# frgfm/Holocron

Measured on NVIDIA H100. Metric: images/sec RepVGG-A0 224^2 bf16 train, higher is better.
Workload: dtype bf16

## Files before the change

holocron_b200/csrc/conv_common.cuh:

```cuda
#pragma once
#include <cuda_runtime.h>
#include <type_traits>
#include "common.cuh"
#include "tc_common.cuh"
#include "tmap.cuh"

namespace conv {

constexpr int kThreads = 384;
constexpr int kConsumers = 256;

__device__ __forceinline__ void consumer_sync() { asm volatile("bar.sync 1, 256;" ::: "memory"); }

struct Ring {
  int stage = 0;
  uint32_t phase = 0;
  __device__ __forceinline__ void next(int n) {
    if (++stage == n) { stage = 0; phase ^= 1; }
  }
  __device__ __forceinline__ static Ring at(int k, int n) { return Ring{k % n, (uint32_t)(k / n) & 1}; }
};

__device__ __forceinline__ void add_residual16(uint4& val, const uint4& rv, bool relu) {
  __nv_bfloat162* a = reinterpret_cast<__nv_bfloat162*>(&val);
  const __nv_bfloat162* b = reinterpret_cast<const __nv_bfloat162*>(&rv);
#pragma unroll
  for (int jj = 0; jj < 4; ++jj) {
    float2 fa = __bfloat1622float2(a[jj]), fb = __bfloat1622float2(b[jj]);
    fa.x += fb.x; fa.y += fb.y;
    if (relu) { fa.x = hb::relu_nan(fa.x); fa.y = hb::relu_nan(fa.y); }
    a[jj] = __floats2bfloat162_rn(fa.x, fa.y);
  }
}

__device__ __forceinline__ void accum_pair(float4& s, const uint8_t* staged) {
  const float2 f = __bfloat1622float2(*reinterpret_cast<const __nv_bfloat162*>(staged));
  s.x += f.x; s.y += f.y; s.z = fmaf(f.x, f.x, s.z); s.w = fmaf(f.y, f.y, s.w);
}
__device__ __forceinline__ float2 fold_stats(const float4* scratch, int rgs, int npairs, int c) {
  const int pr = c >> 1, hi = c & 1;
  float sv = 0.f, qv = 0.f;
  for (int rg = 0; rg < rgs; ++rg) {
    const float4 v = scratch[rg * npairs + pr];
    sv += hi ? v.y : v.x;
    qv += hi ? v.w : v.z;
  }
  return make_float2(sv, qv);
}
__device__ __forceinline__ void store_stats(float* stats, int slot, int Cout, int channel, float2 v) {
  *reinterpret_cast<float2*>(stats + ((size_t)slot * Cout + channel) * 2) = v;
}

template <auto kKernel, typename... Args>
cudaError_t launch(int grid, size_t smem_bytes, cudaStream_t stream, const Args&... args) {
  static const cudaError_t attr =
      cudaFuncSetAttribute(kKernel, cudaFuncAttributeMaxDynamicSharedMemorySize, 227 * 1024);
  if (attr != cudaSuccess) return attr;
  kKernel<<<grid, kThreads, smem_bytes, stream>>>(args...);
  g_hb_launches.fetch_add(1, std::memory_order_relaxed);
  return cudaGetLastError();
}

template <int kStep, int kMax, int W = kStep, typename F>
cudaError_t dispatch_width(int w, F&& f) {
  if (w == W) return f(std::integral_constant<int, W>{});
  if constexpr (W + kStep <= kMax) return dispatch_width<kStep, kMax, W + kStep>(w, f);
  else return cudaErrorInvalidValue;
}

}

int hb_conv_rows_try(const void* x, const void* w, void* y, const float* bias, const void* residual, int N, int H, int W,
                     int Cin, int Cout, int act, int num_ctas, cudaStream_t stream, int nextra, const void* const* xe,
                     const void* const* we, float* stats, int* stat_slots);
int hb_wgrad_rows_try(const void* x, const void* dy, const void* dy1, float* ws, size_t ws_bytes, int N, int H, int W,
                      int Cin, int Cout, int num_ctas, cudaStream_t stream, int* slices_out);
size_t hb_wgrad_rows_workspace_bytes(int N, int H, int W, int Cin, int Cout, int R, int S, int stride, int pad, int dil,
                                     int num_ctas, int has_b1);
```

holocron_b200/csrc/conv_fprop.cu:

```cuda
#include <stdlib.h>
#include "conv_common.cuh"
#include "holocron_b200.h"

namespace {

using namespace tc;
using namespace conv;

constexpr int kBM = 128;
constexpr int kBK = 64;
constexpr int kMmaK = 16;
constexpr int kProducerRegs = 40;
constexpr int kConsumerRegs = 232;
constexpr int kABytes = kBM * kBK * 2;
constexpr int kSmemMax = 227 * 1024;

struct FpropParams {
  int m_total;
  int Ho, Wo;
  int stride, pad_h, pad_w, dil;
  int R, S;
  int Cin, Cout;
  int num_m_tiles, num_n_tiles;
  int cblocks;
// ... 322 lines not shown
  p.e_mode = kext ? 1 : (dual ? 2 : 0);
  const int ce = kext ? a.Ce : (dual ? Cin : 0);
  p.e_cblocks = (ce + kBK - 1) / kBK;
  p.e_ksteps_last = p.e_cblocks ? ((ce - (p.e_cblocks - 1) * kBK) + kMmaK - 1) / kMmaK : 0;
  p.b_stage_bytes = ((BN * 128) + 1023) & ~1023;
  p.out_pitch = (BN < 64 ? BN : 64) * 2 + 16;
  const int out_bytes = ((((kBM * p.out_pitch + 15) & ~15) + kBM * 8) + 1023) & ~1023;
  const int stage_bytes = kABytes + p.b_stage_bytes;
  int stages = (kSmemMax - 1024 - out_bytes - 2 * 8 * (int)sizeof(uint64_t)) / stage_bytes;
  if (stages > 8) stages = 8;
  if (stages < 2) return (int)cudaErrorInvalidValue;
  p.stages = stages;
  p.a_mode = (R == 1 && S == 1 && a.stride == 1 && a.pad_h == 0 && a.pad_w == 0 && a.pad_after_h == 0 &&
              a.pad_after_w == 0) ? 0 : 1;
  p.act = a.act;
  p.y = (__nv_bfloat16*)a.y;
  p.y2 = (__nv_bfloat16*)a.y2;
  p.stats = a.stats; p.stats2 = dual ? a.stats2 : nullptr;
  p.bias = a.bias;
  p.residual = (const __nv_bfloat16*)a.residual;
  p.norm_mean = a.norm_mean; p.norm_rstd = a.norm_rstd; p.norm_wsum = a.norm_wsum;
  if (p.norm_mean && (!p.norm_rstd || !p.norm_wsum || a.scatter)) return (int)cudaErrorInvalidValue;

  CUtensorMap tmA, tmB, tmA2, tmB2;
  int rc = p.a_mode == 0 ? tmap::encode_matrix(&tmA, a.x, p.m_total, Cin, kBM)
                         : tmap::encode_im2col_bf16(&tmA, a.x, a.N, a.H, a.W, Cin, a.pad_h, a.pad_w, R, S, a.dil,
                                                    a.stride, kBK, kBM, CU_TENSOR_MAP_SWIZZLE_128B, a.pad_after_h,
                                                    a.pad_after_w);
  if (rc) return rc;
  if ((rc = tmap::encode_krsc_slab(&tmB, a.w, Cout, R * S, Cin, BN))) return rc;
  tmA2 = tmA; tmB2 = tmB;
  if (kext && (rc = tmap::encode_matrix(&tmA2, a.xe, p.m_total, a.Ce, kBM))) return rc;
  if (p.e_mode && (rc = tmap::encode_krsc_slab(&tmB2, kext ? a.we : a.w2, Cout, 1, ce, BN))) return rc;

  const size_t smem_bytes = (size_t)stages * stage_bytes + out_bytes + 2 * stages * sizeof(uint64_t) + 1024;
  int per_n = grid / p.num_n_tiles;
  if (per_n < 1) per_n = 1;
  if (per_n > p.num_m_tiles) per_n = p.num_m_tiles;
  grid = per_n * p.num_n_tiles;
  if (a.stat_slots) *a.stat_slots = 2 * per_n;
  const bool stats = p.stats || p.stats2;
  return (int)dispatch_width<16, 256>(BN, [&](auto bn) {
    constexpr int kBN = decltype(bn)::value;
    if constexpr (kBN > 128) {
      if (stats) return cudaErrorInvalidValue;
      return launch<conv_fprop_kernel<false, kBN>>(grid, smem_bytes, a.stream, tmA, tmB, tmA2, tmB2, p);
    } else {
      return stats ? launch<conv_fprop_kernel<true, kBN>>(grid, smem_bytes, a.stream, tmA, tmB, tmA2, tmB2, p)
                   : launch<conv_fprop_kernel<false, kBN>>(grid, smem_bytes, a.stream, tmA, tmB, tmA2, tmB2, p);
    }
  });
}

}

extern "C" {

int hb_conv2d_fprop_bf16(const void* x, const void* w, void* y, const float* bias, const void* residual, int N, int H,
                         int W, int Cin, int Cout, int R, int S, int stride, int pad, int dil, int act, int num_ctas,
                         void* stream) {
  hb_conv_args a{};
  a.x = x; a.w = w; a.y = y; a.bias = bias; a.residual = residual;
  a.N = N; a.H = H; a.W = W; a.Cin = Cin; a.Cout = Cout; a.R = R; a.S = S; a.stride = stride; a.pad = pad; a.dil = dil;
  a.act = act; a.num_ctas = num_ctas;
  return hb_conv2d_fused_bf16(&a, nullptr, stream);
}

int hb_conv_stat_slots_max(void) { return 2 * HB_NUM_SMS * 4; }

int hb_conv2d_fused_bf16(const hb_conv_args* c, int* stat_slots, void* stream) {
  if (!c) return (int)cudaErrorInvalidValue;
  const int N = c->N, H = c->H, W = c->W, Cin = c->Cin, Cout = c->Cout, R = c->R, S = c->S;
  const int stride = c->stride, pad = c->pad, dil = c->dil;
  if (Cin % 8 != 0 || Cout % 16 != 0) return (int)cudaErrorInvalidValue;
  if (!hb::aligned16(c->x) || !hb::aligned16(c->w) || !hb::aligned16(c->y)) return (int)cudaErrorMisalignedAddress;
  if (c->w2 && (!hb::aligned16(c->w2) || !hb::aligned16(c->y2))) return (int)cudaErrorMisalignedAddress;
  const int Ho = (H + 2 * pad - dil * (R - 1) - 1) / stride + 1;
  const int Wo = (W + 2 * pad - dil * (S - 1) - 1) / stride + 1;
  if (Ho <= 0 || Wo <= 0) return (int)cudaErrorInvalidValue;
  if ((long long)N * Ho * Wo > 0x7fffffffLL) return (int)cudaErrorInvalidValue;
  if (c->w2 && pad != (R / 2) * dil) return (int)cudaErrorInvalidValue;
  if ((c->stats || c->stats2) && !stat_slots) return (int)cudaErrorInvalidValue;

  if (R == 3 && S == 3 && stride == 1 && pad == 1 && dil == 1 && !c->xe && !c->w2 && !c->norm_mean) {
    static const bool rows_enabled = getenv("HB_DISABLE_CONV_ROWS") == nullptr;
    if (rows_enabled) {
      const int rc = hb_conv_rows_try(c->x, c->w, c->y, c->bias, c->residual, N, H, W, Cin, Cout, c->act, c->num_ctas,
                                      (cudaStream_t)stream, 0, nullptr, nullptr, c->stats, stat_slots);
      if (rc != (int)cudaErrorNotSupported) return rc;
    }
  }
  FpropArgs a{};
  a.x = c->x; a.w = c->w; a.y = c->y; a.bias = c->bias; a.residual = c->residual;
  a.N = N; a.H = H; a.W = W; a.Cin = Cin; a.Cout = Cout; a.R = R; a.S = S; a.stride = stride;
  a.pad_h = a.pad_w = a.pad_after_h = a.pad_after_w = pad; a.dil = dil; a.act = c->act; a.num_ctas = c->num_ctas;
  a.Ho = Ho; a.Wo = Wo; a.stream = (cudaStream_t)stream;
  a.xe = c->xe; a.we = c->we; a.Ce = c->Ce; a.w2 = c->w2; a.y2 = c->y2;
  a.stats = c->stats; a.stats2 = c->stats2; a.stat_slots = stat_slots;
  a.norm_mean = c->norm_mean; a.norm_rstd = c->norm_rstd; a.norm_wsum = c->norm_wsum;
  return fprop_launch(a);
}

int hb_conv2d_dgrad_s2_bf16(const void* dy, const void* wcls, const void* dy1, const void* wd1, void* dx, int N, int H, int W,
                            int Ho, int Wo, int C, int Cd, int num_ctas, void* stream) {
  if (C % 8 != 0 || Cd % 16 != 0) return (int)cudaErrorInvalidValue;
  if (!hb::aligned16(dy) || !hb::aligned16(wcls) || !hb::aligned16(dx)) return (int)cudaErrorMisalignedAddress;
  if (Ho != (H - 1) / 2 + 1 || Wo != (W - 1) / 2 + 1 || H < 2 || W < 2) return (int)cudaErrorInvalidValue;
  const __nv_bfloat16* wc = (const __nv_bfloat16*)wcls;
  size_t woff = 0;
  for (int a = 0; a < 2; ++a) {
    for (int b = 0; b < 2; ++b) {
      const int Hc = (H - a + 1) / 2, Wc = (W - b + 1) / 2;
      const int R = 1 + a, S = 1 + b;
      FpropArgs f{};
      f.x = dy; f.w = wc + woff; f.y = dx; f.bias = nullptr; f.residual = nullptr;
      f.N = N; f.H = Ho; f.W = Wo; f.Cin = C; f.Cout = Cd; f.R = R; f.S = S; f.stride = 1;
      f.pad_h = 0; f.pad_w = 0;
      f.pad_after_h = a ? Hc + 1 - Ho : 0;
      f.pad_after_w = b ? Wc + 1 - Wo : 0;
      f.dil = 1; f.act = 0; f.num_ctas = num_ctas;
      f.Ho = Hc; f.Wo = Wc;
      f.scatter = 1; f.OH = H; f.OW = W; f.o_step = 2; f.o_a = a; f.o_b = b;
      f.stream = (cudaStream_t)stream;
      if (a == 0 && b == 0 && dy1 && wd1) {
        FpropArgs g = f;
        g.x = dy1; g.w = wd1;
        if (int rc = fprop_launch(g)) return rc;
        f.residual = dx;
      }
      if (Hc > 0 && Wc > 0) {
        if (int rc = fprop_launch(f)) return rc;
      }
      woff += (size_t)Cd * R * S * C;
    }
  }
  return 0;
}

}
```

holocron_b200/csrc/conv_rows.cu:

```cuda
#include "conv_common.cuh"

namespace {

using namespace tc;
using namespace conv;

struct RowsParams {
  int N, H, W, Cin, Cout;
  int Wp;
  int SR;
  int NSUB;
  int TRO;
  int CB;
  int ksteps_last;
  int tiles_per_img, num_tiles;
  int nstages;
  int stage_bytes;
  int cb_bytes;
  int ecb_bytes;
  int w_tap_bytes;
  int out_pitch;
  int act;
  int nextra;
  __nv_bfloat16* y;
  const float* bias;
  const __nv_bfloat16* residual;
  float* stats;
};

template <int BN>
__global__ void __launch_bounds__(kThreads, 1)
conv_rows_kernel(const __grid_constant__ CUtensorMap tmX, const __grid_constant__ CUtensorMap tmW,
                 const __grid_constant__ CUtensorMap tmXe0, const __grid_constant__ CUtensorMap tmWe0,
                 const __grid_constant__ CUtensorMap tmXe1, const __grid_constant__ CUtensorMap tmWe1, const RowsParams p) {
  extern __shared__ __align__(1024) uint8_t smem_raw[];
  uint8_t* smem = reinterpret_cast<uint8_t*>((reinterpret_cast<uintptr_t>(smem_raw) + 1023) & ~uintptr_t(1023));
  uint8_t* wsm = smem;
  uint8_t* stage0 = wsm + (size_t)(9 + p.nextra) * p.CB * p.w_tap_bytes;
  uint8_t* sout = stage0 + (size_t)p.nstages * p.stage_bytes;
  const size_t sout_bytes = ((size_t)128 * p.out_pitch + 15) & ~size_t(15);
  uint64_t* bars = reinterpret_cast<uint64_t*>(sout + sout_bytes);
  uint64_t* full_bar = bars;
  uint64_t* empty_bar = bars + 2;
  uint64_t* w_bar = bars + 4;

  const int warp = threadIdx.x >> 5, lane = threadIdx.x & 31;
  if (warp == 0 && lane == 0) {
    prefetch_tmap(&tmX);
    prefetch_tmap(&tmW);
    for (int i = 0; i < 2; ++i) { mbar_init(&full_bar[i], 1); mbar_init(&empty_bar[i], kConsumers / 32); }
    mbar_init(w_bar, 1);
    fence_barrier_init();
  }
  __syncthreads();

  if (warp < 4) {
    if (warp == 0 && lane == 0) {
      prefetch_tmap(&tmXe0); prefetch_tmap(&tmWe0); prefetch_tmap(&tmXe1); prefetch_tmap(&tmWe1);
      mbar_arrive_expect_tx(w_bar, (uint32_t)((9 + p.nextra) * p.CB * BN * 128));
      for (int tap = 0; tap < 9; ++tap)
        for (int cb = 0; cb < p.CB; ++cb)
          tma_load_3d(&tmW, w_bar, wsm + (size_t)(tap * p.CB + cb) * p.w_tap_bytes, cb * 64, tap, 0);
      for (int e = 0; e < p.nextra; ++e)
        for (int cb = 0; cb < p.CB; ++cb)
          tma_load_3d(e == 0 ? &tmWe0 : &tmWe1, w_bar, wsm + (size_t)((9 + e) * p.CB + cb) * p.w_tap_bytes, cb * 64, 0, 0);
      const uint32_t tx = (uint32_t)(p.CB * ((p.TRO + 2) + p.nextra * p.TRO) * p.Wp * 128);
      int it = 0;
      for (int tile = blockIdx.x; tile < p.num_tiles; tile += gridDim.x, ++it) {
        const int n = tile / p.tiles_per_img, p0 = (tile % p.tiles_per_img) * p.TRO;
        const Ring ring = Ring::at(it, p.nstages);
        mbar_wait(&empty_bar[ring.stage], ring.phase ^ 1);
        mbar_arrive_expect_tx(&full_bar[ring.stage], tx);
        for (int b = 0; b <= p.nextra; ++b) {
          const CUtensorMap* tm = b == 0 ? &tmX : (b == 1 ? &tmXe0 : &tmXe1);
          const int h0 = b == 0 ? p0 - 1 : p0;
          for (int cb = 0; cb < p.CB; ++cb) {
            tma_load_4d(tm, &full_bar[ring.stage],
                        stage0 + (size_t)ring.stage * p.stage_bytes +
                            (size_t)p.CB * (b ? p.cb_bytes + (b - 1) * p.ecb_bytes : 0) +
                            (size_t)cb * (b ? p.ecb_bytes : p.cb_bytes),
                        cb * 64, -1, h0, n);
          }
        }
      }
    }
    return;
  }

  const int et = threadIdx.x - 128;
  const int wg = et >> 7;
  const int frow = 64 * wg + frag_row(et & 127);
  const int fcol = frag_col(et & 127);
  const uint32_t dhi = desc_hi(1024);
  const uint32_t w_lo0 = desc_lo(smem_u32(wsm), 16);
  const uint32_t w_tap_lo = (uint32_t)p.w_tap_bytes >> 4;
  const uint32_t cb_lo = (uint32_t)p.cb_bytes >> 4;
  const uint32_t ecb_lo = (uint32_t)p.ecb_bytes >> 4;
  const int chunks_per_row = BN / 8;
  const int npairs = BN >> 1, rgs = kConsumers / npairs;
  const int st_rg = et / npairs, st_pr = et - st_rg * npairs;
  const bool st_on = p.stats != nullptr && st_rg < rgs;
  float4 stat = make_float4(0.f, 0.f, 0.f, 0.f);
  float acc[64];
  mbar_wait(w_bar, 0);
  int it = 0;
  for (int tile = blockIdx.x; tile < p.num_tiles; tile += gridDim.x, ++it) {
    const int n = tile / p.tiles_per_img, p0 = (tile % p.tiles_per_img) * p.TRO;
    const Ring ring = Ring::at(it, p.nstages);
    mbar_wait(&full_bar[ring.stage], ring.phase);
    const uint32_t s_lo =
        desc_lo(smem_u32(stage0 + (size_t)ring.stage * p.stage_bytes), 16) + (uint32_t)wg * ((64 * 128) >> 4);
    for (int sub = 0; sub < p.NSUB; ++sub) {
#pragma unroll 1
      for (int tap = 0; tap < 9; ++tap) {
        const int r = tap / 3, s = tap % 3;
        uint32_t a_lo = s_lo + (uint32_t)(((sub * p.SR + r) * p.Wp + s) * 8);
        uint32_t b_lo = w_lo0 + (uint32_t)(tap * p.CB) * w_tap_lo;
        for (int cb = 0; cb < p.CB; ++cb) {
          const int ks = (cb == p.CB - 1) ? p.ksteps_last : 4;
          wgmma_group_ks<BN, 0, 0>(ks, acc, a_lo, b_lo, 2, dhi, (tap | cb) ? 1u : 0u);
          a_lo += cb_lo;
          b_lo += w_tap_lo;
        }
      }
      for (int e = 0; e < p.nextra; ++e) {
        uint32_t a_lo = s_lo + (uint32_t)p.CB * (cb_lo + e * ecb_lo) + (uint32_t)((sub * p.SR * p.Wp + 1) * 8);
        uint32_t b_lo = w_lo0 + (uint32_t)((9 + e) * p.CB) * w_tap_lo;
        for (int cb = 0; cb < p.CB; ++cb) {
          const int ks = (cb == p.CB - 1) ? p.ksteps_last : 4;
          wgmma_group_ks<BN, 0, 0>(ks, acc, a_lo, b_lo, 2, dhi, 1u);
          a_lo += ecb_lo;
          b_lo += w_tap_lo;
        }
      }
      wgmma_wait<0>();
      fence_regs(acc);
      if (sub == p.NSUB - 1 && lane == 0) mbar_arrive(&empty_bar[ring.stage]);

      consumer_sync();
#pragma unroll
      for (int j = 0; j < 16; ++j) {
        const int col = 8 * j + fcol;
        if (col < BN) {
#pragma unroll
          for (int h = 0; h < 2; ++h) {
            float f0 = acc[4 * j + 2 * h], f1 = acc[4 * j + 2 * h + 1];
            if (p.bias) { f0 += __ldg(p.bias + col); f1 += __ldg(p.bias + col + 1); }
            if (p.act == 1 && !p.residual) { f0 = hb::relu_nan(f0); f1 = hb::relu_nan(f1); }
            *reinterpret_cast<__nv_bfloat162*>(sout + (size_t)(frow + 8 * h) * p.out_pitch + col * 2) =
                __floats2bfloat162_rn(f0, f1);
          }
        }
      }
      consumer_sync();
      const int row0 = p0 + sub * p.SR;
      const int rows_valid = max(0, min(p.SR, min(p.H, p0 + p.TRO) - row0));
      const int total = rows_valid * p.W * chunks_per_row;
      int pix0 = et / chunks_per_row;
      int c8 = et - pix0 * chunks_per_row;
      int i = pix0 / p.W, q = pix0 - i * p.W;
      const int dpix = kConsumers / chunks_per_row, dc = kConsumers - dpix * chunks_per_row;
      const int di = dpix / p.W, dq = dpix - di * p.W;
      for (int ch = et; ch < total; ch += kConsumers) {
        uint4 val = *reinterpret_cast<const uint4*>(sout + (size_t)(i * p.Wp + q) * p.out_pitch + c8 * 16);
        const size_t off = ((size_t)(n * p.H + row0 + i) * p.W + q) * p.Cout + c8 * 8;
        if (p.residual) {
          const uint4 rv = *reinterpret_cast<const uint4*>(p.residual + off);
          add_residual16(val, rv, p.act == 1);
        }
        *reinterpret_cast<uint4*>(p.y + off) = val;
        c8 += dc; q += dq; i += di;
        if (c8 >= chunks_per_row) { c8 -= chunks_per_row; ++q; }
        if (q >= p.W) { q -= p.W; ++i; }
      }
      if (st_on && !p.residual) {
        const int npix = rows_valid * p.W;
        int si = st_rg / p.W, sq = st_rg - si * p.W;
        const int sdi = rgs / p.W, sdq = rgs - sdi * p.W;
        const uint8_t* sp = sout + st_pr * 4;
        for (int v = st_rg; v < npix; v += rgs) {
          accum_pair(stat, sp + (size_t)(si * p.Wp + sq) * p.out_pitch);
          sq += sdq; si += sdi;
          if (sq >= p.W) { sq -= p.W; ++si; }
        }
      }
    }
  }
  if (p.stats) {
    consumer_sync();
    float4* scratch = reinterpret_cast<float4*>(sout);
    scratch[et] = stat;
    consumer_sync();
    if (et < 2 * BN) {
      const int c = et % BN, half = et / BN;
      store_stats(p.stats, blockIdx.x * 2 + half, p.Cout, c,
                  half == 0 ? fold_stats(scratch, rgs, npairs, c) : make_float2(0.f, 0.f));
    }
  }
}

}

int hb_conv_rows_try(const void* x, const void* w, void* y, const float* bias, const void* residual, int N, int H, int W,
                     int Cin, int Cout, int act, int num_ctas, cudaStream_t stream, int nextra, const void* const* xe,
                     const void* const* we, float* stats, int* stat_slots) {
  constexpr int kNo = (int)cudaErrorNotSupported;
  if (stats && (residual || !stat_slots)) return kNo;
  if (Cout % 16 != 0 || Cout > 128 || Cin % 8 != 0 || Cin > 128) return kNo;
  const int Wp = W + 2;
  if (Wp > 128 || W < 8 || nextra < 0 || nextra > 2) return kNo;
  RowsParams p{};
  p.N = N; p.H = H; p.W = W; p.Cin = Cin; p.Cout = Cout; p.Wp = Wp; p.nextra = nextra;
  p.SR = 128 / Wp;
  p.CB = (Cin + 63) / 64;
  const int last = Cin - (p.CB - 1) * 64;
  p.ksteps_last = (last + 15) / 16;
  p.w_tap_bytes = ((Cout * 128) + 1023) & ~1023;
  p.out_pitch = Cout * 2 + 16;
  const int w_bytes = (9 + nextra) * p.CB * p.w_tap_bytes;
  const int out_bytes = (((128 * p.out_pitch + 15) & ~15) + 1023) & ~1023;
  const int budget = 222 * 1024 - w_bytes - out_bytes - 256;
  const int max_rows_needed = (H + p.SR - 1) / p.SR;
  int nsub = 0;
  for (int nst = 2; nst >= 1 && nsub < 1; --nst) {
    for (nsub = max_rows_needed < 8 ? max_rows_needed : 8; nsub >= 1; --nsub) {
      const int tro = nsub * p.SR;
      const int reach = (((nsub - 1) * p.SR + 2) * Wp + 2 + 128) * 128;
      const int rows = (tro + 2) * Wp * 128;
      const int need = ((rows > reach ? rows : reach) + 1023) & ~1023;
      const int ereach = ((nsub - 1) * p.SR * Wp + 1 + 128) * 128, erows = tro * Wp * 128;
      const int eneed = ((erows > ereach ? erows : ereach) + 1023) & ~1023;
      if (nst * p.CB * (need + nextra * eneed) <= budget) {
        p.nstages = nst; p.cb_bytes = need; p.ecb_bytes = eneed;
        break;
      }
    }
  }
  if (nsub < 1) return kNo;
  p.NSUB = nsub;
  p.TRO = nsub * p.SR;
  p.stage_bytes = p.CB * (p.cb_bytes + nextra * p.ecb_bytes);
  p.tiles_per_img = (H + p.TRO - 1) / p.TRO;
  p.num_tiles = N * p.tiles_per_img;
  p.act = act;
  p.y = (__nv_bfloat16*)y; p.bias = bias; p.residual = (const __nv_bfloat16*)residual;
  p.stats = stats;

  CUtensorMap tmX, tmW, tmXe[2], tmWe[2];
  if (tmap::encode_nhwc_box(&tmX, x, N, H, W, Cin, Wp, p.TRO + 2)) return kNo;
  if (tmap::encode_krsc_slab(&tmW, w, Cout, 9, Cin, Cout)) return kNo;
  for (int e = 0; e < 2; ++e) {
    const void* xs = e < nextra ? xe[e] : x;
    const void* ws = e < nextra ? we[e] : w;
    if (!hb::aligned16(xs) || !hb::aligned16(ws)) return kNo;
    if (tmap::encode_nhwc_box(&tmXe[e], xs, N, H, W, Cin, Wp, p.TRO)) return kNo;
    if (tmap::encode_krsc_slab(&tmWe[e], ws, Cout, 1, Cin, Cout)) return kNo;
  }
  const size_t smem_bytes = (size_t)w_bytes + (size_t)p.nstages * p.stage_bytes + out_bytes + 64 + 1024;
  if (smem_bytes > 227 * 1024) return kNo;
  int grid = num_ctas > 0 ? num_ctas : HB_NUM_SMS;
  if (grid > p.num_tiles) grid = p.num_tiles;
  if (stat_slots) *stat_slots = 2 * grid;
  return (int)dispatch_width<16, 128>(Cout, [&](auto bn) {
    return launch<conv_rows_kernel<decltype(bn)::value>>(grid, smem_bytes, stream, tmX, tmW, tmXe[0], tmWe[0], tmXe[1],
                                                          tmWe[1], p);
  });
}

extern "C" {

int hb_conv3x3_accum_bf16(const void* x, const void* w, const void* xe0, const void* we0, const void* xe1, const void* we1,
                          int nextra, void* y, int N, int H, int W, int Cin, int Cout, int num_ctas, void* stream) {
  const void* xe[2] = {xe0, xe1};
  const void* we[2] = {we0, we1};
  if (!hb::aligned16(x) || !hb::aligned16(w) || !hb::aligned16(y)) return (int)cudaErrorMisalignedAddress;
  return hb_conv_rows_try(x, w, y, nullptr, nullptr, N, H, W, Cin, Cout, 0, num_ctas, (cudaStream_t)stream, nextra, xe, we,
                          nullptr, nullptr);
}

}
```

holocron_b200/nn/_fused.py:

```python
import ctypes
import functools
import os
import weakref
from typing import List, Optional, Sequence, Tuple

import torch
from torch import Tensor, nn

from .._lib import DTYPE_CODE, ConvArgs, check, dtype_code, lib, ptr, require_cuda, stream_ptr

ACT_NONE, ACT_RELU, ACT_RELU6, ACT_SILU, ACT_LEAKY, ACT_MISH, ACT_HARDMISH, ACT_FRELU = range(8)

_c_float = ctypes.c_float
_VP3 = ctypes.c_void_p * 3

KERNEL_TIMER = None


def _timed(kind: str, info: dict, fn):
    if KERNEL_TIMER is None:
        return fn()
    e0, e1 = torch.cuda.Event(enable_timing=True), torch.cuda.Event(enable_timing=True)
    e0.record()
    rc = fn()
    e1.record()
    if rc == 0:
        KERNEL_TIMER.append((kind, info, e0, e1))
    return rc


def conv_work(m_out: int, cout: int, k_total: int, in_elems: int, w_elems: int, out_elems: Optional[int] = None,
              w_bytes_per: int = 2) -> dict:
    out_elems = m_out * cout if out_elems is None else out_elems
    return {"flops": 2.0 * m_out * cout * k_total, "bytes": 2.0 * (in_elems + out_elems) + w_bytes_per * w_elems}


@functools.lru_cache(maxsize=None)
def _sm_count(index: int) -> int:
    return torch.cuda.get_device_properties(index).multi_processor_count


def conv_stat_slots(device) -> int:
    return 2 * _sm_count(torch.device(device).index or 0)


def bn_stat_slots(device) -> int:
    return 4 * _sm_count(torch.device(device).index or 0)


def epilogue_stats_pay_off(k_total: int) -> bool:
    if os.environ.get("HB_DISABLE_CONV_STATS"):
        return False
    if os.environ.get("HB_FORCE_CONV_STATS"):
        return True
    return k_total >= 1024


def attach_stats(t: Tensor, parts: Tensor, slots: int) -> None:
    t._hb_stats = (parts, int(slots), t._version)


def get_stats(t: Tensor):
    st = getattr(t, "_hb_stats", None)
    if st is None or st[2] != t._version or st[0].shape[1] != t.shape[1] or st[1] < 1:
        return None
    return st[0], st[1]


def direct_grad(p: Tensor, krsc: bool = False) -> Optional[Tensor]:
    if not getattr(p, "_hb_direct_grad", False):
        return None
    g = p.grad
    if g is None or g.dtype != torch.float32 or g.shape != p.shape or not g.is_cuda:
        return None
    if krsc:
        if g.ndim != 4 or not g.permute(0, 2, 3, 1).is_contiguous():
            return None
    elif not g.is_contiguous():
        return None
    return g


def act_code(act: Optional[nn.Module]) -> Tuple[int, float]:
    if act is None or isinstance(act, nn.Identity):
        return ACT_NONE, 0.0
    if isinstance(act, nn.ReLU6):
        return ACT_RELU6, 0.0
    if isinstance(act, nn.ReLU):
        return ACT_RELU, 0.0
    if isinstance(act, nn.SiLU):
        return ACT_SILU, 0.0
    if isinstance(act, nn.LeakyReLU):
        return ACT_LEAKY, float(act.negative_slope)
    if isinstance(act, nn.Mish):
        return ACT_MISH, 0.0
    if type(act).__name__ == "HardMish":
        return ACT_HARDMISH, 0.0
    raise NotImplementedError(f"no fused kernel for activation {type(act).__name__}")


def round_up(v: int, m: int) -> int:
    return (v + m - 1) // m * m


def to_channels_last_bf16(x: Tensor, c_pad: Optional[int] = None) -> Tensor:
    require_cuda(x)
    n, c, h, w = x.shape
    cp = c if c_pad is None else c_pad
    if cp == c and x.dtype == torch.bfloat16 and x.is_contiguous(memory_format=torch.channels_last):
        return x
    no_grad = not (x.requires_grad and torch.is_grad_enabled())
    if no_grad and x.is_contiguous() and x.dtype in (torch.float32, torch.bfloat16, torch.float16) and (cp != c or c < 8):
        out = torch.empty((n, cp, h, w), device=x.device, dtype=torch.bfloat16).contiguous(memory_format=torch.channels_last)
        check(lib().hb_nchw_to_nhwc_pad_bf16(ptr(x), ptr(out), n, c, h, w, cp, dtype_code(x), stream_ptr()),
              "hb_nchw_to_nhwc_pad_bf16")
        return out
    y = x.to(torch.bfloat16).contiguous(memory_format=torch.channels_last)
    if cp != c:
        out = torch.zeros((n, cp, h, w), device=x.device, dtype=torch.bfloat16).contiguous(memory_format=torch.channels_last)
        out[:, :c] = y
        return out
    return y


def _empty_cl(n: int, c: int, h: int, w: int, device, dtype=torch.bfloat16) -> Tensor:
    return torch.empty((n, c, h, w), device=device, dtype=dtype, memory_format=torch.channels_last)


class PackedFilter:
    __slots__ = ("wf", "wd", "key", "cin_p", "cout_p", "cin_d", "cout", "cin", "r", "s", "wref", "w_krsc", "need_dgrad")


_pack_cache = {}


class _PackTable:

    def __init__(self) -> None:
# ... 475 lines not shown
            raise NotImplementedError("fused BN kernels need channels % 8 == 0")
        m = n * h * w
        dev = us[0].device if nb else res.device
        c_log = gammas[0].numel() if nb else c
        stats = _bn_setup(us, branches, gammas, betas, training, c, c_log, m, dev)
        out = _bn_forward_pass(us, stats, res, m, c, act, slope, int(res_after), (n, c, h, w), emit_stats)
        ctx.save_for_backward(stats, *us, *([res] if has_res else []), *gammas, *betas)
        ctx.cfg = (nb, act, slope, training, has_res, c_log, int(res_after))
        return out

    @staticmethod
    def backward(ctx, dout: Tensor):
        nb, act, slope, training, has_res, c_log, res_after = ctx.cfg
        saved = ctx.saved_tensors
        stats, us = saved[0], saved[1:1 + nb]
        res = saved[1 + nb] if has_res else None
        params = saved[1 + nb + int(has_res):]
        gammas, betas = params[:nb], params[nb:]
        n, c, h, w = us[0].shape if nb else res.shape
        m = n * h * w
        dev = dout.device
        dob = to_channels_last_bf16(dout)
        need_u = [ctx.needs_input_grad[1 + i] for i in range(nb)]
        need_gb = any(ctx.needs_input_grad[1 + nb:1 + 3 * nb])
        need_res = has_res and ctx.needs_input_grad[1 + 3 * nb]
        dus = [_empty_cl(n, c, h, w, dev) if need_u[i] else None for i in range(nb)]
        dres = _empty_cl(n, c, h, w, dev) if need_res else None
        gacc, bacc, dgb = _bn_grad_targets(gammas, betas, c, dev) if need_gb else (None, None, None)
        _bn_backward_pass(dob, us, stats, res, dus, dres, dgb, gacc, bacc, c_log, m, c, act, slope, training, res_after)
        grads: List[Optional[Tensor]] = [None]
        grads += dus
        grads += [dgb[0][i][:c_log] if dgb is not None else None for i in range(nb)]
        grads += [dgb[1][i][:c_log] if dgb is not None else None for i in range(nb)]
        if has_res:
            grads.append(dres)
        return tuple(grads)


def bn_act(us: Sequence[Tensor], bns: Sequence[nn.BatchNorm2d], act: int = ACT_NONE, slope: float = 0.0,
           residual: Optional[Tensor] = None, training: Optional[bool] = None, res_after_act: bool = False,
           emit_stats: bool = False) -> Tensor:
    if not 1 <= len(us) <= 3 or len(us) != len(bns):
        raise ValueError("between 1 and 3 (input, BatchNorm2d) pairs are supported")
    require_cuda(*us)
    if training is None:
        training = bns[0].training
    use_batch_stats = training or bns[0].running_mean is None
    cfg = ([BNBranch(b) for b in bns], int(act), float(slope), bool(use_batch_stats), residual is not None,
           bool(res_after_act), bool(emit_stats))
    args = list(us) + [b.weight for b in bns] + [b.bias for b in bns]
    if residual is not None:
        args.append(residual)
    return _BNActFn.apply(cfg, *args)


def act_only(x: Tensor, act: int, slope: float = 0.0) -> Tensor:
    cfg = ([], int(act), float(slope), False, True, False, False)
    return _BNActFn.apply(cfg, x)


class _RepBlockFn(torch.autograd.Function):

    @staticmethod
    def forward(ctx, cfg, x: Tensor, w3: Tensor, w1: Tensor, *bn_params: Tensor) -> Tensor:
        branches, act, slope, training, stride = cfg
        nb = len(branches)
        gammas, betas = bn_params[:nb], bn_params[nb:]
        need_dx = ctx.needs_input_grad[1]
        cout, cin = w3.shape[0], w3.shape[1]
        if cout % 16 != 0:
            raise NotImplementedError("fused RepBlock needs out_channels % 16 == 0")
        stem = cin <= 4 and x.shape[1] == cin and not need_dx and x.is_contiguous() and x.dtype in DTYPE_CODE
        if stem:
            xb, wf3, wf1 = _stem_im2col(x, w3, stride, w1)
            k3, conv_stride, pad3 = 1, 1, 0
            wd3 = wd1 = None
        else:
            pk3 = pack_filter(w3, need_dx, round_up(x.shape[1], 8))
            pk1 = pack_filter(w1, need_dx, round_up(x.shape[1], 8))
            xb = to_channels_last_bf16(x, pk3.cin_p)
            wf3, wf1, wd3, wd1 = pk3.wf, pk1.wf, pk3.wd, pk1.wd
            k3, conv_stride, pad3 = 3, stride, 1
        kx = xb.shape[1]
        if os.environ.get("HB_FUSED_FPROP"):
            y3, y1 = conv2d_forward_raw(xb, wf3, cout, k3, k3, conv_stride, pad3, 1, w2=wf1,
                                        want_stats=training and epilogue_stats_pay_off(k3 * k3 * kx))
        else:
            y3 = conv2d_forward_raw(xb, wf3, cout, k3, k3, conv_stride, pad3, 1,
                                    want_stats=training and epilogue_stats_pay_off(k3 * k3 * kx))
            y1 = conv2d_forward_raw(xb, wf1, cout, 1, 1, conv_stride, 0, 1,
                                    want_stats=training and epilogue_stats_pay_off(kx))
        us = [y3, y1] + ([xb] if nb == 3 else [])
        n, c, h, w = y3.shape
        m = n * h * w
        stats = _bn_setup(us, branches, gammas, betas, training, c, c, m, y3.device)
        out = _bn_forward_pass(us, stats, None, m, c, act, slope, 0, (n, c, h, w), emit_stats=training)
        ctx.save_for_backward(stats, xb, y3, y1, w3, w1, *gammas, *betas)
        ctx.cfg = (nb, act, slope, training, stride, wd3, wd1, x.shape[1], stem)
        return out

    @staticmethod
    def backward(ctx, dout: Tensor):
        nb, act, slope, training, stride, wd3, wd1, cin_x, stem = ctx.cfg
        stats, xb, y3, y1, w3, w1 = ctx.saved_tensors[:6]
        gammas, betas = ctx.saved_tensors[6:6 + nb], ctx.saved_tensors[6 + nb:6 + 2 * nb]
        n, c, ho, wo = y3.shape
        _, cin_p, h, w = xb.shape
        m = n * ho * wo
        dev = dout.device
        L = lib()
        dob = to_channels_last_bf16(dout)
        need_dx = ctx.needs_input_grad[1]
        dy3, dy1 = _empty_cl(n, c, ho, wo, dev), _empty_cl(n, c, ho, wo, dev)
        dxid = _empty_cl(n, c, ho, wo, dev) if (nb == 3 and need_dx) else None
        gacc, bacc, dgb = _bn_grad_targets(gammas, betas, c, dev)
        us = [y3, y1] + ([xb] if nb == 3 else [])
        _bn_backward_pass(dob, us, stats, None, [dy3, dy1] + ([dxid] if nb == 3 else []), None, dgb, gacc, bacc, c, m, c, act,
                          slope, training, 0)
        g_gamma = [None if dgb is None else dgb[0][i] for i in range(nb)]
        g_beta = [None if dgb is None else dgb[1][i] for i in range(nb)]
        dx = None
        if need_dx:
            cin_d = wd3.shape[0]
            if stride == 1 and wd3.shape[3] == c and (dxid is None or cin_d == c):
                dxp = None
                if not os.environ.get("HB_DISABLE_CONV_ROWS"):
                    eye = _identity_filter(cin_d, c, dev) if dxid is not None else None
                    dxr = _empty_cl(n, cin_d, h, w, dev)
                    nsrc = 2 if dxid is not None else 1
                    info = dict(shape=("dgrad_rows", h, c, cin_d, 3, 1), launches=1,
                                **conv_work(n * h * w, cin_d, 10 * c, (1 + nsrc) * n * h * w * c, 10 * cin_d * c))
                    rc = _timed("dgrad", info, lambda: L.hb_conv3x3_accum_bf16(
                        ptr(dy3), ptr(wd3), ptr(dy1), ptr(wd1), ptr(dxid), ptr(eye), nsrc, ptr(dxr), n, h, w, c, cin_d, 0,
                        stream_ptr()))
                    if rc == 0:
                        dxp = dxr
                    elif rc != 801:
                        check(rc, "hb_conv3x3_accum_bf16")
                if dxp is None:
                    dxp = conv2d_forward_raw(dy3, wd3, cin_d, 3, 3, 1, 1, 1, None, dxid, ACT_NONE, xe=dy1, we=wd1, kind="dgrad")
            else:
                dxp = _dgrad(dy3, w3, wd3, cin_d, h, w, stride, 1, dy1, wd1)
                if dxid is not None:
                    dxp[:, :c].add_(dxid)
            dx = dxp if cin_d == cin_x else dxp[:, :cin_x]
        if stem:
            return (None, None, _stem_wgrad(xb, dy3, w3), _stem_wgrad(xb, dy1, w1), *g_gamma, *g_beta)
        grads_w: List[Optional[Tensor]] = [None, None]
        done = [False, False]
        no_pad = cin_p == w3.shape[1]
        gw3 = direct_grad(w3, krsc=True) if no_pad else None
        gw1 = direct_grad(w1, krsc=True) if no_pad else None
        if stride == 1 and not os.environ.get("HB_DISABLE_FUSED_WGRAD"):
            ws_bytes = L.hb_repvgg_wgrad_workspace_bytes(n, h, w, cin_p, c, 0)
            if ws_bytes:
                ws = torch.empty(ws_bytes // 4, device=dev, dtype=torch.float32)
                info = dict(shape=("wgrad_rows", h, cin_p, c, 3, 1), launches=2,
                            **conv_work(n * h * w, c, 10 * cin_p, n * h * w * (cin_p + 2 * c), 10 * c * cin_p, out_elems=0,
                                        w_bytes_per=4))
                if gw3 is not None and gw1 is not None:
                    rc = _timed("wgrad", info, lambda: L.hb_repvgg_wgrad_acc_bf16(
                        ptr(xb), ptr(dy3), ptr(dy1), ptr(gw3), ptr(gw1), ptr(ws), ws_bytes, n, h, w, cin_p, c, 0, stream_ptr()))
                    if rc == 0:
                        done = [True, True]
                    elif rc != 801:
                        check(rc, "hb_repvgg_wgrad_acc_bf16")
                else:
                    dwcat = torch.empty(c * 10 * cin_p, device=dev, dtype=torch.float32)
                    rc = _timed("wgrad", info, lambda: L.hb_repvgg_wgrad_bf16(
# ... 117 lines not shown
```

Before: 7880.

## Fuse 1x1 branch into rows 3x3 conv kernel for dual-output RepVGG fprop

Extends the row-tiled 3x3 conv kernel with a dual mode that also computes the 1x1 branch from the same staged input tile (center tap), writing a second output and optional second stats. The RepBlock forward now uses the fused dual path by default when Cout <= 64, instead of only under an env flag. This removes a second launch and a second read of the input for the 1x1 conv. The cost is higher register pressure from the extra accumulator and a second epilogue pass per subtile. The dual path requests epilogue stats only when both branches qualify, so small-Cin layers may lose in-kernel stats.

```diff
diff --git a/holocron_b200/csrc/conv_common.cuh b/holocron_b200/csrc/conv_common.cuh
--- a/holocron_b200/csrc/conv_common.cuh
+++ b/holocron_b200/csrc/conv_common.cuh
@@ -72,7 +72,7 @@
 
 int hb_conv_rows_try(const void* x, const void* w, void* y, const float* bias, const void* residual, int N, int H, int W,
                      int Cin, int Cout, int act, int num_ctas, cudaStream_t stream, int nextra, const void* const* xe,
-                     const void* const* we, float* stats, int* stat_slots);
+                     const void* const* we, float* stats, int* stat_slots, const void* w2, void* y2, float* stats2);
 int hb_wgrad_rows_try(const void* x, const void* dy, const void* dy1, float* ws, size_t ws_bytes, int N, int H, int W,
                       int Cin, int Cout, int num_ctas, cudaStream_t stream, int* slices_out);
 size_t hb_wgrad_rows_workspace_bytes(int N, int H, int W, int Cin, int Cout, int R, int S, int stride, int pad, int dil,
diff --git a/holocron_b200/csrc/conv_fprop.cu b/holocron_b200/csrc/conv_fprop.cu
--- a/holocron_b200/csrc/conv_fprop.cu
+++ b/holocron_b200/csrc/conv_fprop.cu
@@ -428,11 +428,12 @@
   if (c->w2 && pad != (R / 2) * dil) return (int)cudaErrorInvalidValue;
   if ((c->stats || c->stats2) && !stat_slots) return (int)cudaErrorInvalidValue;
 
-  if (R == 3 && S == 3 && stride == 1 && pad == 1 && dil == 1 && !c->xe && !c->w2 && !c->norm_mean) {
+  if (R == 3 && S == 3 && stride == 1 && pad == 1 && dil == 1 && !c->xe && !c->norm_mean) {
     static const bool rows_enabled = getenv("HB_DISABLE_CONV_ROWS") == nullptr;
     if (rows_enabled) {
       const int rc = hb_conv_rows_try(c->x, c->w, c->y, c->bias, c->residual, N, H, W, Cin, Cout, c->act, c->num_ctas,
-                                      (cudaStream_t)stream, 0, nullptr, nullptr, c->stats, stat_slots);
+                                      (cudaStream_t)stream, 0, nullptr, nullptr, c->stats, stat_slots, c->w2, c->y2,
+                                      c->stats2);
       if (rc != (int)cudaErrorNotSupported) return rc;
     }
   }
diff --git a/holocron_b200/csrc/conv_rows.cu b/holocron_b200/csrc/conv_rows.cu
--- a/holocron_b200/csrc/conv_rows.cu
+++ b/holocron_b200/csrc/conv_rows.cu
@@ -22,13 +22,16 @@
   int out_pitch;
   int act;
   int nextra;
+  int n1x1;
   __nv_bfloat16* y;
+  __nv_bfloat16* y2;
   const float* bias;
   const __nv_bfloat16* residual;
   float* stats;
+  float* stats2;
 };
 
-template <int BN>
+template <int BN, bool kDual>
 __global__ void __launch_bounds__(kThreads, 1)
 conv_rows_kernel(const __grid_constant__ CUtensorMap tmX, const __grid_constant__ CUtensorMap tmW,
                  const __grid_constant__ CUtensorMap tmXe0, const __grid_constant__ CUtensorMap tmWe0,
@@ -36,7 +39,7 @@
   extern __shared__ __align__(1024) uint8_t smem_raw[];
   uint8_t* smem = reinterpret_cast<uint8_t*>((reinterpret_cast<uintptr_t>(smem_raw) + 1023) & ~uintptr_t(1023));
   uint8_t* wsm = smem;
-  uint8_t* stage0 = wsm + (size_t)(9 + p.nextra) * p.CB * p.w_tap_bytes;
+  uint8_t* stage0 = wsm + (size_t)(9 + p.n1x1) * p.CB * p.w_tap_bytes;
   uint8_t* sout = stage0 + (size_t)p.nstages * p.stage_bytes;
   const size_t sout_bytes = ((size_t)128 * p.out_pitch + 15) & ~size_t(15);
   uint64_t* bars = reinterpret_cast<uint64_t*>(sout + sout_bytes);
@@ -57,11 +60,11 @@
   if (warp < 4) {
     if (warp == 0 && lane == 0) {
       prefetch_tmap(&tmXe0); prefetch_tmap(&tmWe0); prefetch_tmap(&tmXe1); prefetch_tmap(&tmWe1);
-      mbar_arrive_expect_tx(w_bar, (uint32_t)((9 + p.nextra) * p.CB * BN * 128));
+      mbar_arrive_expect_tx(w_bar, (uint32_t)((9 + p.n1x1) * p.CB * BN * 128));
       for (int tap = 0; tap < 9; ++tap)
         for (int cb = 0; cb < p.CB; ++cb)
           tma_load_3d(&tmW, w_bar, wsm + (size_t)(tap * p.CB + cb) * p.w_tap_bytes, cb * 64, tap, 0);
-      for (int e = 0; e < p.nextra; ++e)
+      for (int e = 0; e < p.n1x1; ++e)
         for (int cb = 0; cb < p.CB; ++cb)
           tma_load_3d(e == 0 ? &tmWe0 : &tmWe1, w_bar, wsm + (size_t)((9 + e) * p.CB + cb) * p.w_tap_bytes, cb * 64, 0, 0);
       const uint32_t tx = (uint32_t)(p.CB * ((p.TRO + 2) + p.nextra * p.TRO) * p.Wp * 128);
@@ -99,9 +102,10 @@
   const int chunks_per_row = BN / 8;
   const int npairs = BN >> 1, rgs = kConsumers / npairs;
   const int st_rg = et / npairs, st_pr = et - st_rg * npairs;
-  const bool st_on = p.stats != nullptr && st_rg < rgs;
-  float4 stat = make_float4(0.f, 0.f, 0.f, 0.f);
+  const bool st_on = st_rg < rgs;
+  float4 stat = make_float4(0.f, 0.f, 0.f, 0.f), stat2 = make_float4(0.f, 0.f, 0.f, 0.f);
   float acc[64];
+  float acc1[kDual ? BN / 2 : 1];
   mbar_wait(w_bar, 0);
   int it = 0;
   for (int tile = blockIdx.x; tile < p.num_tiles; tile += gridDim.x, ++it) {
@@ -133,91 +137,111 @@
           b_lo += w_tap_lo;
         }
       }
+      if constexpr (kDual) {
+        uint32_t a_lo = s_lo + (uint32_t)(((sub * p.SR + 1) * p.Wp + 1) * 8);
+        uint32_t b_lo = w_lo0 + (uint32_t)(9 * p.CB) * w_tap_lo;
+        for (int cb = 0; cb < p.CB; ++cb) {
+          const int ks = (cb == p.CB - 1) ? p.ksteps_last : 4;
+          wgmma_group_ks<BN, 0, 0>(ks, acc1, a_lo, b_lo, 2, dhi, cb ? 1u : 0u);
+          a_lo += cb_lo;
+          b_lo += w_tap_lo;
+        }
+      }
       wgmma_wait<0>();
       fence_regs(acc);
+      if constexpr (kDual) fence_regs(acc1);
       if (sub == p.NSUB - 1 && lane == 0) mbar_arrive(&empty_bar[ring.stage]);
 
-      consumer_sync();
-#pragma unroll
-      for (int j = 0; j < 16; ++j) {
-        const int col = 8 * j + fcol;
-        if (col < BN) {
-#pragma unroll
-          for (int h = 0; h < 2; ++h) {
-            float f0 = acc[4 * j + 2 * h], f1 = acc[4 * j + 2 * h + 1];
-            if (p.bias) { f0 += __ldg(p.bias + col); f1 += __ldg(p.bias + col + 1); }
-            if (p.act == 1 && !p.residual) { f0 = hb::relu_nan(f0); f1 = hb::relu_nan(f1); }
-            *reinterpret_cast<__nv_bfloat162*>(sout + (size_t)(frow + 8 * h) * p.out_pitch + col * 2) =
-                __floats2bfloat162_rn(f0, f1);
-          }
-        }
-      }
-      consumer_sync();
       const int row0 = p0 + sub * p.SR;
       const int rows_valid = max(0, min(p.SR, min(p.H, p0 + p.TRO) - row0));
-      const int total = rows_valid * p.W * chunks_per_row;
-      int pix0 = et / chunks_per_row;
-      int c8 = et - pix0 * chunks_per_row;
-      int i = pix0 / p.W, q = pix0 - i * p.W;
-      const int dpix = kConsumers / chunks_per_row, dc = kConsumers - dpix * chunks_per_row;
-      const int di = dpix / p.W, dq = dpix - di * p.W;
-      for (int ch = et; ch < total; ch += kConsumers) {
-        uint4 val = *reinterpret_cast<const uint4*>(sout + (size_t)(i * p.Wp + q) * p.out_pitch + c8 * 16);
-        const size_t off = ((size_t)(n * p.H + row0 + i) * p.W + q) * p.Cout + c8 * 8;
-        if (p.residual) {
-          const uint4 rv = *reinterpret_cast<const uint4*>(p.residual + off);
-          add_residual16(val, rv, p.act == 1);
-        }
-        *reinterpret_cast<uint4*>(p.y + off) = val;
-        c8 += dc; q += dq; i += di;
-        if (c8 >= chunks_per_row) { c8 -= chunks_per_row; ++q; }
-        if (q >= p.W) { q -= p.W; ++i; }
-      }
-      if (st_on && !p.residual) {
-        const int npix = rows_valid * p.W;
-        int si = st_rg / p.W, sq = st_rg - si * p.W;
-        const int sdi = rgs / p.W, sdq = rgs - sdi * p.W;
-        const uint8_t* sp = sout + st_pr * 4;
-        for (int v = st_rg; v < npix; v += rgs) {
-          accum_pair(stat, sp + (size_t)(si * p.Wp + sq) * p.out_pitch);
-          sq += sdq; si += sdi;
-          if (sq >= p.W) { sq -= p.W; ++si; }
-        }
-      }
+      auto epilogue = [&](const float* a, __nv_bfloat16* yo, const float* st_ptr, float4& st, bool first) {
+        consumer_sync();
+#pragma unroll
+        for (int j = 0; j < 16; ++j) {
+          if (8 * j < BN) {
+            const int col = 8 * j + fcol;
+#pragma unroll
+            for (int h = 0; h < 2; ++h) {
+              float f0 = a[4 * j + 2 * h], f1 = a[4 * j + 2 * h + 1];
+              if (first && p.bias) { f0 += __ldg(p.bias + col); f1 += __ldg(p.bias + col + 1); }
+              if (first && p.act == 1 && !p.residual) { f0 = hb::relu_nan(f0); f1 = hb::relu_nan(f1); }
+              *reinterpret_cast<__nv_bfloat162*>(sout + (size_t)(frow + 8 * h) * p.out_pitch + col * 2) =
+                  __floats2bfloat162_rn(f0, f1);
+            }
+          }
+        }
+        consumer_sync();
+        const int total = rows_valid * p.W * chunks_per_row;
+        int pix0 = et / chunks_per_row;
+        int c8 = et - pix0 * chunks_per_row;
+        int i = pix0 / p.W, q = pix0 - i * p.W;
+        const int dpix = kConsumers / chunks_per_row, dc = kConsumers - dpix * chunks_per_row;
+        const int di = dpix / p.W, dq = dpix - di * p.W;
+        for (int ch = et; ch < total; ch += kConsumers) {
+          uint4 val = *reinterpret_cast<const uint4*>(sout + (size_t)(i * p.Wp + q) * p.out_pitch + c8 * 16);
+          const size_t off = ((size_t)(n * p.H + row0 + i) * p.W + q) * p.Cout + c8 * 8;
+          if (first && p.residual) {
+            const uint4 rv = *reinterpret_cast<const uint4*>(p.residual + off);
+            add_residual16(val, rv, p.act == 1);
+          }
+          *reinterpret_cast<uint4*>(yo + off) = val;
+          c8 += dc; q += dq; i += di;
+          if (c8 >= chunks_per_row) { c8 -= chunks_per_row; ++q; }
+          if (q >= p.W) { q -= p.W; ++i; }
+        }
+        if (st_ptr && st_on) {
+          const int npix = rows_valid * p.W;
+          int si = st_rg / p.W, sq = st_rg - si * p.W;
+          const int sdi = rgs / p.W, sdq = rgs - sdi * p.W;
+          const uint8_t* sp = sout + st_pr * 4;
+          for (int v = st_rg; v < npix; v += rgs) {
+            accum_pair(st, sp + (size_t)(si * p.Wp + sq) * p.out_pitch);
+            sq += sdq; si += sdi;
+            if (sq >= p.W) { sq -= p.W; ++si; }
+          }
+        }
+      };
+      epilogue(acc, p.y, p.stats, stat, true);
+      if constexpr (kDual) epilogue(acc1, p.y2, p.stats2, stat2, false);
     }
   }
-  if (p.stats) {
+  auto fold = [&](float* so, const float4& st) {
     consumer_sync();
     float4* scratch = reinterpret_cast<float4*>(sout);
-    scratch[et] = stat;
+    scratch[et] = st;
     consumer_sync();
     if (et < 2 * BN) {
       const int c = et % BN, half = et / BN;
-      store_stats(p.stats, blockIdx.x * 2 + half, p.Cout, c,
+      store_stats(so, blockIdx.x * 2 + half, p.Cout, c,
                   half == 0 ? fold_stats(scratch, rgs, npairs, c) : make_float2(0.f, 0.f));
     }
-  }
+  };
+  if (p.stats) fold(p.stats, stat);
+  if (kDual && p.stats2) fold(p.stats2, stat2);
 }
 
 }
 
 int hb_conv_rows_try(const void* x, const void* w, void* y, const float* bias, const void* residual, int N, int H, int W,
                      int Cin, int Cout, int act, int num_ctas, cudaStream_t stream, int nextra, const void* const* xe,
-                     const void* const* we, float* stats, int* stat_slots) {
+                     const void* const* we, float* stats, int* stat_slots, const void* w2, void* y2, float* stats2) {
   constexpr int kNo = (int)cudaErrorNotSupported;
-  if (stats && (residual || !stat_slots)) return kNo;
+  const bool dual = w2 != nullptr;
+  if (!dual) stats2 = nullptr;
+  if ((stats || stats2) && (residual || !stat_slots)) return kNo;
+  if (dual && (nextra || residual || !y2 || !hb::aligned16(y2) || Cout > 64)) return kNo;
   if (Cout % 16 != 0 || Cout > 128 || Cin % 8 != 0 || Cin > 128) return kNo;
   const int Wp = W + 2;
   if (Wp > 128 || W < 8 || nextra < 0 || nextra > 2) return kNo;
   RowsParams p{};
-  p.N = N; p.H = H; p.W = W; p.Cin = Cin; p.Cout = Cout; p.Wp = Wp; p.nextra = nextra;
+  p.N = N; p.H = H; p.W = W; p.Cin = Cin; p.Cout = Cout; p.Wp = Wp; p.nextra = nextra; p.n1x1 = nextra + (dual ? 1 : 0);
   p.SR = 128 / Wp;
   p.CB = (Cin + 63) / 64;
   const int last = Cin - (p.CB - 1) * 64;
   p.ksteps_last = (last + 15) / 16;
   p.w_tap_bytes = ((Cout * 128) + 1023) & ~1023;
   p.out_pitch = Cout * 2 + 16;
-  const int w_bytes = (9 + nextra) * p.CB * p.w_tap_bytes;
+  const int w_bytes = (9 + p.n1x1) * p.CB * p.w_tap_bytes;
   const int out_bytes = (((128 * p.out_pitch + 15) & ~15) + 1023) & ~1023;
   const int budget = 222 * 1024 - w_bytes - out_bytes - 256;
   const int max_rows_needed = (H + p.SR - 1) / p.SR;
@@ -244,14 +268,15 @@
   p.num_tiles = N * p.tiles_per_img;
   p.act = act;
   p.y = (__nv_bfloat16*)y; p.bias = bias; p.residual = (const __nv_bfloat16*)residual;
-  p.stats = stats;
+  p.y2 = (__nv_bfloat16*)y2;
+  p.stats = stats; p.stats2 = stats2;
 
   CUtensorMap tmX, tmW, tmXe[2], tmWe[2];
   if (tmap::encode_nhwc_box(&tmX, x, N, H, W, Cin, Wp, p.TRO + 2)) return kNo;
   if (tmap::encode_krsc_slab(&tmW, w, Cout, 9, Cin, Cout)) return kNo;
   for (int e = 0; e < 2; ++e) {
     const void* xs = e < nextra ? xe[e] : x;
-    const void* ws = e < nextra ? we[e] : w;
+    const void* ws = e < nextra ? we[e] : (dual && e == 0 ? w2 : w);
     if (!hb::aligned16(xs) || !hb::aligned16(ws)) return kNo;
     if (tmap::encode_nhwc_box(&tmXe[e], xs, N, H, W, Cin, Wp, p.TRO)) return kNo;
     if (tmap::encode_krsc_slab(&tmWe[e], ws, Cout, 1, Cin, Cout)) return kNo;
@@ -259,11 +284,17 @@
   const size_t smem_bytes = (size_t)w_bytes + (size_t)p.nstages * p.stage_bytes + out_bytes + 64 + 1024;
   if (smem_bytes > 227 * 1024) return kNo;
   int grid = num_ctas > 0 ? num_ctas : HB_NUM_SMS;
+  if (dual && p.num_tiles < grid) return kNo;
   if (grid > p.num_tiles) grid = p.num_tiles;
   if (stat_slots) *stat_slots = 2 * grid;
+  if (dual)
+    return (int)dispatch_width<16, 64>(Cout, [&](auto bn) {
+      return launch<conv_rows_kernel<decltype(bn)::value, true>>(grid, smem_bytes, stream, tmX, tmW, tmXe[0], tmWe[0],
+                                                                 tmXe[1], tmWe[1], p);
+    });
   return (int)dispatch_width<16, 128>(Cout, [&](auto bn) {
-    return launch<conv_rows_kernel<decltype(bn)::value>>(grid, smem_bytes, stream, tmX, tmW, tmXe[0], tmWe[0], tmXe[1],
-                                                          tmWe[1], p);
+    return launch<conv_rows_kernel<decltype(bn)::value, false>>(grid, smem_bytes, stream, tmX, tmW, tmXe[0], tmWe[0],
+                                                                tmXe[1], tmWe[1], p);
   });
 }
 
@@ -275,7 +306,7 @@
   const void* we[2] = {we0, we1};
   if (!hb::aligned16(x) || !hb::aligned16(w) || !hb::aligned16(y)) return (int)cudaErrorMisalignedAddress;
   return hb_conv_rows_try(x, w, y, nullptr, nullptr, N, H, W, Cin, Cout, 0, num_ctas, (cudaStream_t)stream, nextra, xe, we,
-                          nullptr, nullptr);
-}
-
-}
+                          nullptr, nullptr, nullptr, nullptr, nullptr);
+}
+
+}
diff --git a/holocron_b200/nn/_fused.py b/holocron_b200/nn/_fused.py
--- a/holocron_b200/nn/_fused.py
+++ b/holocron_b200/nn/_fused.py
@@ -54,6 +54,13 @@
     if os.environ.get("HB_FORCE_CONV_STATS"):
         return True
     return k_total >= 1024
+
+
+def dual_fprop(cout: int) -> bool:
+    force = os.environ.get("HB_FUSED_FPROP")
+    if force:
+        return force != "0"
+    return cout <= 64
 
 
 def attach_stats(t: Tensor, parts: Tensor, slots: int) -> None:
@@ -695,9 +702,10 @@
             wf3, wf1, wd3, wd1 = pk3.wf, pk1.wf, pk3.wd, pk1.wd
             k3, conv_stride, pad3 = 3, stride, 1
         kx = xb.shape[1]
-        if os.environ.get("HB_FUSED_FPROP"):
+        if dual_fprop(cout):
             y3, y1 = conv2d_forward_raw(xb, wf3, cout, k3, k3, conv_stride, pad3, 1, w2=wf1,
-                                        want_stats=training and epilogue_stats_pay_off(k3 * k3 * kx))
+                                        want_stats=training and epilogue_stats_pay_off(k3 * k3 * kx)
+                                        and epilogue_stats_pay_off(kx))
         else:
             y3 = conv2d_forward_raw(xb, wf3, cout, k3, k3, conv_stride, pad3, 1,
                                     want_stats=training and epilogue_stats_pay_off(k3 * k3 * kx))
```

Result: faster. 8035 (median of 6 runs) (+2.0%).
